# liron88/HM-16.2

Measured on AMD Instinct MI355X. Metric: CTUs/sec (enc) at 4K main10; bit-exact CU partition vs HM, higher is better.
Workload: dtype int32+f64

## Files before the change

### hm-16.2_amd/csrc/hm355_core.h

```cpp
#pragma once
#include <stddef.h>
#include "hm355_types.h"

#ifdef HM355_HOSTSIM
#include <string.h>
#include <math.h>
#include <stdlib.h>
#define HM_DEV static
#define HM_NOINLINE __attribute__((noinline))
#define HM_CONST static const
#define HM_ASSUME_LDS(p) ((void)0)
#define HM_ASSUME_GLB(p) ((void)0)
#define HM_NT 1
static inline int hm_lane() { return 0; }
#define HM_SYNC() ((void)0)
static inline uint32_t hm_wave_sum(uint32_t v) { return v; }
static inline int hm_wave_sum_i(int v) { return v; }
static inline int hm_wave_max_i(int v) { return v; }
#define HM_UNI(x) (x)
#define HM_UCALL(x) (x)
#define hm_uni_ptr(p) (p)
#define hm_uni_struct(v) (v)
#define HM_ENTRY(e) ((void)0)
#define HM_LDS_ADD(p, v) (*(p) += (v))
// ... 206 lines not shown
};
struct CuFrame { int16_t cuZ; int8_t phase, sub, boundary, parentPart, ampSens, pad_; double bestCost, splitCost; uint32_t bestBits, bestDist, splitBits, splitDist; };
struct MvFieldD { MvD mv; int ref; };
struct MergeList { MvFieldD f[5][2]; uint8_t dir[5]; int num; };
struct AmvpInfo { MvD cand[3]; int n; };
struct TZ {
  const Pel *org; int orgStride, w, h;
  const Pel *ref; int refStride;
  uint32_t bestSad; int bestX, bestY, bestDist, bestRound, pointNr;
  int16_t l, r, t, b;
  int16_t subShift, pad_;
  int16_t lx[16], ly[16]; int8_t lp[16], ld[16];
  int16_t wx0, wy0, ww, wh;
};
struct IrqFrame {
  TU t; int8_t phase, child, checkFull, checkSplit, zero; uint8_t bestTS[3];
  uint32_t absSum[3], bestCBF[3], singleBits, singleDist, subBits, subDist; double singleCost, subCost;
};

#define HM_TSTRIDE 33
#define HM_RQ_LDS 256
struct RqLds {
  int32_t lvl[HM_RQ_LDS];
  uint16_t pos[HM_RQ_LDS];
  uint16_t dec[HM_RQ_LDS];
  int16_t cur[HM_RQ_LDS];
  uint8_t ctxSig[HM_RQ_LDS];
  uint8_t code[HM_RQ_LDS];
  uint8_t cgCtxSet[64];
  uint8_t cgFlag[64];
};
struct RefLds {
  Pel refTop[2][132], refLeft[2][132];
  Pel refMain[200], refSide[200];
  Pel line[272];
};
#define HM_SLOT(d, ci) ((d) * CI_NUM + (ci) - ((d) == 4 ? 2 : 0))
#define HM_NUM_SLOTS (4 * CI_NUM + 3)
struct Team;
#define HM_CTU_WAVES 12
struct LdsTables {
  int8_t tmat[32 * HM_TSTRIDE];
  int8_t dst4[16];
  int32_t ebits[128];
};
#if defined(HM355_HOSTSIM)
static LdsTables g_lt;
#else
__shared__ LdsTables g_lt;
#endif
#define HM_LT() (&g_lt)
struct Shared {
  Cabac cur;
  int32_t bufA[32 * HM_TSTRIDE];
  union {
    int32_t bufB[32 * HM_TSTRIDE];
    RqLds rq;
    RefLds ref;
  } u;
  TuWalk walkOuter, walkInner;
  CuFrame cuf[4];
  double outCost; uint32_t outBits, outDist; double outRdCost;
  int32_t mpmZ;
  int32_t s8Winner, s8Reuse;
  InterMeta *im;
  uint32_t mcost; MvD mvPredictor; int32_t costScale;
  union {
    struct {
      uint8_t flags[72];
      RqtFrame rqt[4]; uint32_t rqtRetDist[5], rqtRetBits[5]; double rqtRetCost[5];
      int32_t rdModeList[12];
      uint8_t splitCbf[5][2];
      uint32_t outDistY;
      uint32_t satd[36];
      int32_t mpmNum, mpmPreds[3];
    };
    struct {
      int32_t absCoeff[10];
      TZ tz; MvD outMv; MergeList ml; AmvpInfo amvp; MvFieldD mrgField[2]; int32_t mrgDir, mrgIdx; uint32_t mrgCost, irqZeroDist;
      IrqFrame irq[4];
    };
  };
  int32_t width, height, bitDepth, wCtu, stride[3];
  const Params *P; FrameBuf fb; WorkSpace *ws; const Tables *tab;
  CtuMeta meta;
  TCoeff *cc;
  int32_t ctuX, ctuY, ctuAddr;
// ... 7 lines not shown
static FILE *g_hm_trace;
#define HM_TRACE(e, tag, a, b, c) do { if (g_hm_trace) fprintf(g_hm_trace, "%d %d %u %u %.3f\n", (int)(tag), (e)->ctuAddr, (unsigned)(a), (unsigned)(b), (double)(c)); } while (0)
#elif defined(HM355_TRACE)
#define HM_TRACE_CAP (1u << 21)
__device__ inline void hm_trace(Shared *e, int tag, uint32_t a, uint32_t b, double c)
{
  if (hm_lane() == 0) {
    unsigned long long *t = e->P->prof; const unsigned long long n = atomicAdd(t, 1ull);
    if (n < HM_TRACE_CAP) { t[1 + n * 3] = ((unsigned long long)(uint32_t)tag << 32) | (uint32_t)e->ctuAddr; t[2 + n * 3] = ((unsigned long long)a << 32) | b; t[3 + n * 3] = (unsigned long long)__double_as_longlong(c); }
  }
}
#define HM_TRACE(e, tag, a, b, c) hm_trace((e), (tag), (uint32_t)(a), (uint32_t)(b), (double)(c))
#else
#define HM_TRACE(e, tag, a, b, c) ((void)0)
#endif

#ifndef HM355_HOSTSIM
__shared__ Shared g_sh;
__shared__ Shared g_shs[HM_CTU_WAVES];
#endif
#if !defined(HM355_PROFILE)
static_assert(HM_CTU_WAVES * (sizeof(Shared) + 16) + sizeof(LdsTables) <= 163840 / (12 / HM_CTU_WAVES) && sizeof(Shared) % 8 == 0, "two workgroups of HM_CTU_WAVES searches (+ work items, + the shared tables) per CU: 12 CTU searches in 160 KB of LDS");
#endif
static_assert(offsetof(Shared, bufA) % 8 == 0 && (16 * HM_TSTRIDE * 4) % 8 == 0, "the RDOQ cost array aliases the lower half of bufA as doubles");
static_assert(offsetof(Shared, u) == offsetof(Shared, bufA) + sizeof(((Shared *)0)->bufA), "the motion search stages its reference window across bufA and the union behind it");
#define HM_TZ_WIN_SAMPLES ((int)((sizeof(((Shared *)0)->bufA) + sizeof(((Shared *)0)->u)) / sizeof(Pel)))

HM_DEV inline int hm_clip3(int lo, int hi, int v) { return v < lo ? lo : (v > hi ? hi : v); }
HM_DEV inline int hm_abs(int v) { return v < 0 ? -v : v; }
HM_DEV inline int hm_z2r(int z)
{
  const int x = (z & 1) | ((z >> 1) & 2) | ((z >> 2) & 4) | ((z >> 3) & 8);
  const int y = ((z >> 1) & 1) | ((z >> 2) & 2) | ((z >> 3) & 4) | ((z >> 4) & 8);
  return (y << 4) | x;
}
HM_DEV inline int hm_spread4(int v) { return (v & 1) | ((v & 2) << 1) | ((v & 4) << 2) | ((v & 8) << 3); }
HM_DEV inline int hm_r2z(int r) { return hm_spread4(r & 15) | (hm_spread4(r >> 4) << 1); }
HM_DEV inline int hm_log2(int n) { return n >= 64 ? 6 : (n >= 32 ? 5 : (n >= 16 ? 4 : (n >= 8 ? 3 : 2))); }

HM_DEV inline void par_set8(uint8_t *p, int v, int n) { HM_PAR_FOR(i, n) p[i] = (uint8_t)v; HM_SYNC(); }
HM_DEV inline void par_copy8(uint8_t *d, const uint8_t *s, int n) { HM_PAR_FOR(i, n) d[i] = s[i]; HM_SYNC(); }
HM_DEV inline void par_copy32(TCoeff *d, const TCoeff *s, int n) { HM_PAR_FOR(i, n) d[i] = s[i]; HM_SYNC(); }
HM_DEV inline void par_zero32(TCoeff *d, int n) { HM_PAR_FOR(i, n) d[i] = 0; HM_SYNC(); }
HM_DEV inline void par_copy_blk(Pel *d, int ds, const Pel *s, int ss, int n)
{
  const int l2 = hm_log2(n);
// ... 666 lines not shown
  const uint16_t *scan = e->tab->scan[scanType][log2n - 2], *scanCG = e->tab->scanCG[scanType][log2n - 2];
  const int firstCtx = first_sig_ctx(n, scanType, chroma);
  const int sigOff = C_SIG + (chroma ? 28 : 0);
  const int32_t *src = e->bufA;
  WorkSpace *ws = e->ws;
  const bool big = n == 32;
  double *costCoeff = big ? ws->costCoeff : (double *)(e->bufA + 16 * HM_TSTRIDE);
  int32_t *rqLvl = big ? (int32_t *)e->u.bufB : e->u.rq.lvl;
  uint16_t *rqPos = big ? (uint16_t *)e->bufA : e->u.rq.pos, *rqDec = big ? (uint16_t *)e->bufA + 1024 : e->u.rq.dec;
  int16_t *rqCur = e->u.rq.cur;
  uint8_t *rqCtxSig = e->u.rq.ctxSig, *rqCode = e->u.rq.code;
  uint8_t *cgCtxSet = big ? (uint8_t *)e->u.bufB + 4096 : e->u.rq.cgCtxSet;
  int lastLocal = -1;
  {
    const int64_t cap = 2147483647LL - (1LL << (qBits - 1));
    HM_PAR_FOR(sp, numCoef) {
      const int blkPos = scan[sp];
      const int32_t sc = src[(blkPos >> log2n) * HM_TSTRIDE + (blkPos & (n - 1))];
      const int64_t tmpLevel = (int64_t)hm_abs(sc) * quantCoef;
      const int32_t lvl = (int32_t)(tmpLevel < cap ? tmpLevel : cap);
      rqLvl[sp] = (big && sc < 0) ? ~lvl : lvl;
      if (!big) rqPos[sp] = (uint16_t)(blkPos | (sc < 0 ? 0x8000 : 0));
      if (((lvl + (1 << (qBits - 1))) >> qBits) > 0 && sp > lastLocal) lastLocal = sp;
      dst[sp] = 0;
    }
  }
  const int lastScanPos = hm_wave_max_i(lastLocal);
  HM_SYNC();
  if (big && lastScanPos >= 0) {
    HM_PAR_FOR(sp, numCoef) {
      const int32_t v = rqLvl[sp]; const int neg = v < 0;
      rqLvl[sp] = neg ? ~v : v;
      rqPos[sp] = (uint16_t)(scan[sp] | (neg ? 0x8000 : 0));
      rqDec[sp] = 0;
    }
    HM_SYNC();
  }
  if (lastScanPos < 0) return 0;
  int lastOff, lastShift; last_ctx_params(chroma, n, &lastOff, &lastShift);
  HM_LV(int32_t, tSig); HM_LV(int32_t, tOne); HM_LV(int32_t, tLast); HM_LV(int32_t, tMisc); HM_LV(int32_t, tLastCost);
  HM_LV(double, vCGSig);
  HM_WAVE_FOR(k) {
    const int bin = k & 1, c = k >> 1;
    HM_LVK(tSig, k) = c < (chroma ? 16 : 28) ? HM_LT()->ebits[cb->s[sigOff + c] ^ bin] : 0;
    HM_LVK(tOne, k) = c < 30 ? HM_LT()->ebits[cb->s[C_ONE + c] ^ bin] : 0;
    HM_LVK(tLast, k) = c < 30 ? HM_LT()->ebits[cb->s[(c < 15 ? C_LASTX + c : C_LASTY + c - 15) + (chroma ? 15 : 0)] ^ bin] : 0;
    HM_LVK(tMisc, k) = c < 15 ? HM_LT()->ebits[cb->s[c < 4 ? C_SIG_CG + c : (c < 14 ? C_QT_CBF + c - 4 : C_ROOT_CBF)] ^ bin] : 0;
    HM_LVK(tLastCost, k) = 0;
    HM_LVK(vCGSig, k) = 0;
  }
  {
    const int gmax = HM_GROUP_IDX[n - 1];
    int accX = 0, accY = 0;
    for (int g = 0; g <= gmax; g++) {
      const int cx = (lastOff + (g >> lastShift)) * 2, cy = 30 + cx;
      int bx = accX, by = accY;
      if (g < gmax) { bx += HM_LV_GET(tLast, cx); by += HM_LV_GET(tLast, cy); }
      if (g > 3) { bx += 32768 * ((g - 2) >> 1); by += 32768 * ((g - 2) >> 1); }
      HM_LV_SET(tLastCost, g, bx); HM_LV_SET(tLastCost, 16 + g, by);
      accX += HM_LV_GET(tLast, cx + 1); accY += HM_LV_GET(tLast, cy + 1);
    }
// ... 238 lines not shown
              if (lastCG == 1 && lastNZ == k && hm_abs(dv) == 1) costDown -= (4 << 15);
              if (costUp < costDown) { curCost = costUp; curChange = 1; }
              else { curChange = -1; if (k == firstNZ && hm_abs(dv) == 1) curCost = I64MAX; else curCost = costDown; }
            } else {
              curCost = rdFactor * (-(hm_abs(deltaU))) + (1 << 15) + rateIncUp + sigRateDelta;
              curChange = 1;
              if (k < firstNZ) { const uint32_t thissign = (uint32_t)HM_LV_GET(sNeg, k); if (thissign != signbit) curCost = I64MAX; }
            }
            if (curCost < minCostInc) { minCostInc = curCost; finalChange = curChange; minK = k; }
          }
          if (minK >= 0) {
            const int mv = HM_LV_GET(sCur, minK);
            if (mv == 32767 || mv == -32768) finalChange = -1;
            const int nv = HM_LV_GET(sNeg, minK) ? mv - finalChange : mv + finalChange;
            if (big) HM_LV_SET(sCur, minK, nv); else rqCur[subPos + minK] = (int16_t)nv;
          }
        }
      }
      if (big) { HM_WAVE_FOR(k) { if (k < 16) rqDec[subPos + k] = (uint16_t)(int16_t)HM_LVK(sCur, k); } }
      if (lastCG == 1) lastCG = 0;
    }
  }
  HM_SYNC();
  HM_PAR_FOR(sp, lastScanPos + 1) {
    int v;
    if (!big) v = rqCur[sp];
    else if (absSum >= 2) v = (int16_t)rqDec[sp];
    else { const int lv = (sp < bestLastIdxP1 && ((cgMask >> scanCG[sp >> 4]) & 1)) ? (int)rqDec[sp] : 0; v = (rqPos[sp] & 0x8000) ? -lv : lv; }
    dst[rqPos[sp] & 0x3ff] = v;
  }
  HM_SYNC();
  return absSum;
}

struct CabacR { HM_LV(int32_t, st); HM_LV(int32_t, eb0); HM_LV(int32_t, eb1); HM_LV(int32_t, lps); uint64_t frac; };
HM_DEV inline void cabr_load(const Shared *e, CabacR &r, const Cabac *c)
{
  HM_WAVE_FOR(k) {
    HM_LVK(r.st, k) = k < (int)(sizeof(c->s) / 4) ? ((const int32_t *)c->s)[k] : 0;
    HM_LVK(r.eb0, k) = HM_LT()->ebits[k]; HM_LVK(r.eb1, k) = HM_LT()->ebits[64 + k];
    HM_LVK(r.lps, k) = ((const int32_t *)HM_NEXT_LPS)[k & 31];
  }
  r.frac = c->frac;
}
HM_DEV inline void cabr_store(const CabacR &r, Cabac *c)
{
// ... 1 lines not shown
  c->frac = r.frac;
  HM_SYNC();
}
HM_DEV inline void enc_bin(const Shared *e, CabacR *r, int ctx, int bin)
{
  const int w = HM_LV_GET(r->st, ctx >> 2), sh = (ctx & 3) * 8, s = (w >> sh) & 0xff, i = s ^ bin;
  const int b0 = HM_LV_GET(r->eb0, i & 63), b1 = HM_LV_GET(r->eb1, i & 63);
  r->frac += (uint64_t)(uint32_t)(i < 64 ? b0 : b1);
  const int lw = HM_LV_GET(r->lps, s >> 2);
  const int ns = (bin == (s & 1)) ? (s < 124 ? s + 2 : s) : ((lw >> ((s & 3) * 8)) & 0xff);
  HM_LV_SET(r->st, ctx >> 2, (w & ~(0xff << sh)) | (ns << sh));
}
HM_DEV inline void enc_ep(CabacR *r, int n) { r->frac += (uint64_t)32768 * (uint64_t)n; }
HM_DEV inline void enc_epv(Cabac *c, uint32_t val, int n) { (void)val; enc_ep(c, n); }
HM_DEV inline void enc_epv(CabacR *r, uint32_t val, int n) { (void)val; enc_ep(r, n); }
#include "hm355_bits.h"
HM_DEV inline int hm_min_in_group(int g) { return g < 4 ? g : ((2 + (g & 1)) << ((g >> 1) - 1)); }

#if defined(HM355_PROFILE) && !defined(HM355_HOSTSIM)
#define HM_BPROF(id) do { if (real) { const unsigned long long t_ = __builtin_readcyclecounter(); e->prof[id] += t_ - profT1; e->profCnt[id] += 1; profT1 = t_; } } while (0)
#else
#define HM_BPROF(id) ((void)0)
#endif
template <class C> HM_DEV HM_NOINLINE void code_coeff_nxn(Shared *e, C *c, const TCoeff *coef, int n, int comp, int scanType, int tskipFlag)
{
  HM_ENTRY(e); n = HM_UNI(n); comp = HM_UNI(comp); scanType = HM_UNI(scanType); tskipFlag = HM_UNI(tskipFlag); c = hm_uni_ptr(c); HM_ASSUME_LDS(c); coef = hm_uni_ptr(coef);
  const int chroma = comp != 0, log2n = hm_log2(n), wg = n >> 2;
  const bool real = EngOf<C>::REAL != 0;
#if defined(HM355_PROFILE) && !defined(HM355_HOSTSIM)
  const unsigned long long profT0 = __builtin_readcyclecounter();
#endif
  typename EngOf<C>::R r; cabr_load(e, r, c);
  if (n == 4) enc_bin(e, &r, C_TSKIP + chroma, tskipFlag);
  const uint16_t *scan = e->tab->scan[scanType][log2n - 2], *scanCG = e->tab->scanCG[scanType][log2n - 2];
  int16_t *lv = (n == 32) ? (int16_t *)e->bufA : e->u.rq.cur; uint8_t *cgFlag = e->u.rq.cgFlag;
  uint16_t *sposArr = (n == 32) ? (uint16_t *)e->bufA + 1024 : e->u.rq.pos;
  HM_PAR_FOR(i, 64) cgFlag[i] = 0;
  HM_SYNC();
  int lastLocal = -1;
  HM_PAR_FOR(sp, n * n) {
    const int blkPos = scan[sp]; const TCoeff v = coef[blkPos];
    lv[sp] = (int16_t)v; sposArr[sp] = (uint16_t)blkPos;
    if (v != 0) { if (sp > lastLocal) lastLocal = sp; const int py = blkPos >> log2n, px = blkPos - (py << log2n); cgFlag[wg * (py >> 2) + (px >> 2)] = 1; }
  }
  const int scanPosLast = hm_wave_max_i(lastLocal);
  HM_SYNC();
#if defined(HM355_PROFILE) && !defined(HM355_HOSTSIM)
  if (real) { e->prof[PR_ADI] += __builtin_readcyclecounter() - profT0; e->profCnt[PR_ADI] += 1; }
  unsigned long long profT1 = __builtin_readcyclecounter();
#endif
  uint64_t cgMask = 0;
  HM_LV(int32_t, vScanCG);
  HM_WAVE_FOR(k) { HM_BALLOT(cgMask, k, cgFlag[k] != 0); HM_LVK(vScanCG, k) = k < wg * wg ? scanCG[k] : 0; }
  const int posLast = sposArr[scanPosLast];
  {
    int py = posLast >> log2n, px = posLast - (py << log2n);
    if (scanType == SCAN_VER) { const int t = px; px = py; py = t; }
    const int gx = hm_group_idx(px), gy = hm_group_idx(py), gmax = hm_group_idx(n - 1);
    int off, shift; last_ctx_params(chroma, n, &off, &shift);
    const int bxc = C_LASTX + (chroma ? 15 : 0) + off, byc = C_LASTY + (chroma ? 15 : 0) + off;
    int k;
    for (k = 0; k < gx; k++) enc_bin(e, &r, bxc + (k >> shift), 1);
    if (gx < gmax) enc_bin(e, &r, bxc + (k >> shift), 0);
    for (k = 0; k < gy; k++) enc_bin(e, &r, byc + (k >> shift), 1);
    if (gy < gmax) enc_bin(e, &r, byc + (k >> shift), 0);
    if (gx > 3) enc_epv(&r, (uint32_t)(px - hm_min_in_group(gx)), (gx - 2) >> 1);
    if (gy > 3) enc_epv(&r, (uint32_t)(py - hm_min_in_group(gy)), (gy - 2) >> 1);
  }
  HM_BPROF(PR_INV);
  const int firstCtx = first_sig_ctx(n, scanType, chroma), sigOff = C_SIG + (chroma ? 28 : 0);
  const int lastScanSet = scanPosLast >> 4;
  int c1 = 1;
  for (int subSet = lastScanSet; subSet >= 0; subSet--) {
    const int subPos = subSet << 4, isLastSet = subSet == lastScanSet;
    const int cgBlkPos = HM_LV_GET(vScanCG, subSet), cgy = cgBlkPos >> (log2n - 2), cgx = cgBlkPos & (wg - 1);
    const int sigRight = (cgx < wg - 1) ? (int)((cgMask >> (cgBlkPos + 1)) & 1) : 0;
    const int sigLower = (cgy < wg - 1) ? (int)((cgMask >> (cgBlkPos + wg)) & 1) : 0;
    if (isLastSet || subSet == 0) cgMask |= 1ull << cgBlkPos;
    else enc_bin(e, &r, C_SIG_CG + (chroma ? 2 : 0) + ((sigRight + sigLower) != 0), (int)((cgMask >> cgBlkPos) & 1));
    if (!((cgMask >> cgBlkPos) & 1)) continue;
    const int pattern = wg <= 1 ? 0 : sigRight + (sigLower << 1);
    const int top = isLastSet ? (scanPosLast & 15) : 15;
    HM_LV(int32_t, vCtx); HM_LV(int32_t, vAbs);
    uint64_t nz = 0, g1 = 0, g2 = 0, ng = 0;
    HM_WAVE_FOR(k) {
      const int kk = k & 15, sp = subPos + kk;
      const int a = (kk <= top) ? hm_abs((int)lv[sp]) : 0;
      if (real) HM_BALLOT(ng, k, kk <= top && lv[sp] < 0 && k < 16);
      HM_LVK(vAbs, k) = a;
      HM_LVK(vCtx, k) = sig_ctx_inc(pattern, firstCtx, sposArr[sp], log2n, chroma);
      HM_BALLOT(nz, k, a != 0 && k < 16); HM_BALLOT(g1, k, a > 1 && k < 16); HM_BALLOT(g2, k, a > 2 && k < 16);
    }
    HM_BPROF(PR_SATD35);
    {
      int seen = isLastSet ? 1 : 0;
      for (int p = isLastSet ? top - 1 : 15; p >= 0; p--) {
        const int sig = (int)((nz >> p) & 1);
        if (p > 0 || subSet == 0 || seen) enc_bin(e, &r, sigOff + HM_LV_GET(vCtx, p), sig);
        seen += sig;
      }
    }
    HM_BPROF(PR_TUBLK);
    const int numNonZero = __builtin_popcountll(nz);
    if (numNonZero > 0) {
      const int lastNZ = 63 - __builtin_clzll(nz), firstNZ = __builtin_ctzll(nz);
      const int signHidden = (lastNZ - firstNZ >= 4);
      const int ctxSet = ctx_set_index(chroma, subSet, c1 == 0);
      c1 = 1;
      int firstC2 = -1, escape = 0, idx = 0;
      for (uint64_t m = nz; m && idx < 8; idx++) {
        const int p = 63 - __builtin_clzll(m); m &= ~(1ull << p);
        const int sym = (int)((g1 >> p) & 1);
        enc_bin(e, &r, C_ONE + 4 * ctxSet + c1, sym);
// ... 170 lines not shown
    enc_subdiv_cbf_qt(e, &r, t, bLuma, bChroma);
    cabr_store(r, &e->cur);
  }
  if (bLuma) enc_coeff_qt(e, t, 0);
  if (bChroma) { enc_coeff_qt(e, t, 1); enc_coeff_qt(e, t, 2); }
  HM_PROF_END(e, PR_BITS);
  return num_bits(&e->cur);
}

HM_DEV HM_NOINLINE uint32_t intra_coding_tu_block(Shared *e, TU tv, int comp, int save1load2)
{
  HM_ENTRY(e); comp = HM_UNI(comp); save1load2 = HM_UNI(save1load2); tv = hm_uni_struct(tv);
  const TU *t = &tv;
  CtuMeta *m = (&e->meta); WorkSpace *ws = e->ws;
  if (comp && !t->cW) return 0;
  const int n = comp ? t->cW : (1 << t->log2), l2 = hm_log2(n);
  const int relZ = comp ? t->cRelZ : t->relZ, z = t->cuZ + relZ;
  const int bx = comp ? t->cx : t->x, by = comp ? t->cy : t->y;
  const int st = HM_PLANE_STRIDE(comp), po = HM_PLANE_OFF(comp);
  const int layer = 5 - t->log2, parts = comp ? t->cParts : t->parts;
  const int ps = e->stride[comp], bitDepth = e->bitDepth;
  const Pel *org = e->fb.org[comp] + (e->ctuY * st + by) * ps + e->ctuX * st + bx;
  Pel *recPic = e->fb.rec[comp] + (e->ctuY * st + by) * ps + e->ctuX * st + bx;
  Pel *pred = ws->pred + po + by * st + bx, *resi = ws->resi + po + by * st + bx;
  Pel *recQt = ws->qtRec[layer] + po + by * st + bx;
  TCoeff *coef = ws->qtCoef[layer] + po + (comp ? t->cOff : z * 16);
  const int tskip = m->ts[comp][z];
  int mode = comp ? m->dirC[z] : m->dirL[z];
  if (comp && mode == DM_CHROMA_IDX) mode = m->dirL[z & ~3];
  if (save1load2 != 2) {
    const int filt = use_filtered_refs(comp, mode, n);
    const int r = hm_z2r(z);
    { HM_PROF_BEGIN(e, PR_ADI); init_adi_pattern(e, comp, e->ctuX * st + bx, e->ctuY * st + by, n, e->ctuX * 16 + (r & 15), e->ctuY * 16 + (r >> 4), comp ? n / 2 : n / 4, filt); HM_PROF_END(e, PR_ADI); }
    { HM_PROF_BEGIN(e, PR_PRED); pred_intra(e, comp, mode, n, filt, pred, st); HM_PROF_END(e, PR_PRED); }
    if (save1load2 == 1) { HM_PAR_FOR(i, 16) e->ws->tsPred[comp][i] = pred[(i >> 2) * st + (i & 3)]; HM_SYNC(); }
  } else { HM_PAR_FOR(i, 16) pred[(i >> 2) * st + (i & 3)] = e->ws->tsPred[comp][i]; HM_SYNC(); }
  if (comp == 0) par_set8(m->tr + z, t->trDepth, parts);
  const int tshift = 15 - bitDepth - l2;
  HM_PAR_FOR(i, n * n) {
    const int y = i >> l2, x = i & (n - 1);
    const int r = org[y * ps + x] - pred[y * st + x];
    resi[y * st + x] = (Pel)r;
    e->bufA[y * HM_TSTRIDE + x] = tskip ? (r << tshift) : r;
  }
  HM_SYNC();
  { HM_PROF_BEGIN(e, PR_FWD); if (!tskip) fwd_transform(e, n, comp == 0 && n == 4, bitDepth); HM_PROF_END(e, PR_FWD); }
  const int cbfCtx = comp ? 5 + t->trDepth : (t->trDepth == 0 ? 1 : 0);
  HM_PROF_BEGIN(e, PR_RDOQ);
  const int absSum = rdoq_is_empty(e, n, comp) ? 0 : (int)HM_UCALL(rdoq(e, coef, n, comp, coef_scan_idx(m, z, n, comp), cbfCtx));
  HM_PROF_END(e, PR_RDOQ);
#if defined(HM355_PROFILE) && !defined(HM355_HOSTSIM)
  { const int pid = l2 == 2 ? (absSum ? 13 : 7) : (l2 == 3 ? 14 : (l2 == 4 ? 15 : 43)); e->prof[pid] += __builtin_readcyclecounter() - prof_t0_PR_RDOQ; e->profCnt[pid] += 1; }
#endif
  par_set8(m->cbf[comp] + z, (absSum > 0 ? 1 : 0) << t->trDepth, parts);
  HM_PROF_BEGIN(e, PR_INV);
  if (absSum > 0) {
    const int rightShift = 6 - (tshift + e->fb.qpPer[comp != 0]);
    const int scale = HM_INV_QUANT_SCALES[e->fb.qpRem[comp != 0]];
    int tgt = 25 + rightShift; if (tgt > 16) tgt = 16;
    const int imin = -(1 << (tgt - 1)), imax = (1 << (tgt - 1)) - 1;
    HM_PAR_FOR(i, n * n) {
      const int y = i >> l2, x = i & (n - 1);
      const int c = hm_clip3(imin, imax, coef[i]);
      int v;
      if (rightShift > 0) v = (c * scale + (1 << (rightShift - 1))) >> rightShift;
      else v = (int)((unsigned)(c * scale) << (-rightShift));
      e->bufA[y * HM_TSTRIDE + x] = hm_clip3(-32768, 32767, v);
    }
    HM_SYNC();
    if (!tskip) inv_transform(e, n, comp == 0 && n == 4, bitDepth);
    const int off = tshift == 0 ? 0 : (1 << (tshift - 1));
    HM_PAR_FOR(i, n * n) {
      const int y = i >> l2, x = i & (n - 1);
      const int v = e->bufA[y * HM_TSTRIDE + x];
      resi[y * st + x] = (Pel)(tskip ? ((v + off) >> tshift) : v);
    }
  } else {
    HM_PAR_FOR(i, n * n) { const int y = i >> l2, x = i & (n - 1); coef[i] = 0; resi[y * st + x] = 0; }
  }
  HM_SYNC();
  HM_PROF_END(e, PR_INV);
  const int maxv = (1 << bitDepth) - 1, shiftSse = (bitDepth - 8) << 1;
  uint32_t sse = 0;
  HM_PAR_FOR(i, n * n) {
    const int y = i >> l2, x = i & (n - 1);
    const int r = hm_clip3(0, maxv, pred[y * st + x] + resi[y * st + x]);
    pred[y * st + x] = (Pel)r; recQt[y * st + x] = (Pel)r; recPic[y * ps + x] = (Pel)r;
    const int d = org[y * ps + x] - r; sse += (uint32_t)((d * d) >> shiftSse);
  }
  uint32_t d = hm_wave_sum(sse);
  HM_SYNC();
  if (comp) d = (uint32_t)(e->fb.chromaWeight * (double)d);
  return d;
}

HM_DEV inline void store_intra_result_qt(Shared *e, const TU *t, int comp)
{
  const int st = HM_PLANE_STRIDE(comp), po = HM_PLANE_OFF(comp), layer = 5 - t->log2;
  const int bx = comp ? t->cx : t->x, by = comp ? t->cy : t->y;
  const TCoeff *coef = e->ws->qtCoef[layer] + po + (comp ? t->cOff : (t->cuZ + t->relZ) * 16);
  const Pel *rq = e->ws->qtRec[layer] + po + by * st + bx;
  HM_PAR_FOR(i, 16) { e->ws->tsCoef[comp][i] = coef[i]; e->ws->tsRec[comp][i] = rq[(i >> 2) * st + (i & 3)]; }
  HM_SYNC();
}
HM_DEV inline void load_intra_result_qt(Shared *e, const TU *t, int comp)
{
  const int st = HM_PLANE_STRIDE(comp), po = HM_PLANE_OFF(comp), layer = 5 - t->log2, ps = e->stride[comp];
  const int bx = comp ? t->cx : t->x, by = comp ? t->cy : t->y;
  TCoeff *coef = e->ws->qtCoef[layer] + po + (comp ? t->cOff : (t->cuZ + t->relZ) * 16);
  Pel *rq = e->ws->qtRec[layer] + po + by * st + bx;
  Pel *recPic = e->fb.rec[comp] + (e->ctuY * st + by) * ps + e->ctuX * st + bx;
  HM_PAR_FOR(i, 16) { coef[i] = e->ws->tsCoef[comp][i]; const Pel v = e->ws->tsRec[comp][i]; rq[(i >> 2) * st + (i & 3)] = v; recPic[(i >> 2) * ps + (i & 3)] = v; }
  HM_SYNC();
}

HM_DEV HM_NOINLINE void simt4_luma_leaf(Shared *e, TU tv);
// ... 4 lines not shown
  CtuMeta *m = (&e->meta);
  RqtFrame *fr = e->rqt; int sp = 0;
  uint32_t *retDist = e->rqtRetDist, *retBits = e->rqtRetBits; double *retCost = e->rqtRetCost;
  fr[0].t = rootv; fr[0].phase = 0; retDist[0] = 0; retBits[0] = 0; retCost[0] = 0.0;
  while (sp >= 0) {
    RqtFrame *f = &fr[sp]; const TU *t = &f->t;
    const int z = t->cuZ + t->relZ, fullDepth = t->cuDepth + t->trDepth, log2 = t->log2;
    if (f->phase == 0) {
      const int nxn = m->part[t->cuZ] == SIZE_NxN;
      f->checkFull = log2 <= 5;
      f->checkSplit = log2 > tr_min_size_in_cu(6 - t->cuDepth, nxn);
      if (checkFirst && f->checkFull) f->checkSplit = 0;
      f->singleCost = HM_MAX_DOUBLE; f->singleDist = 0; f->singleCbf = 0; f->bestModeId = 0; f->singleBits = 0;
      const int checkTS = (log2 == 2) && (m->part[z] == SIZE_NxN);
      if (f->checkFull) {
        if (checkTS) {
          cabac_copy(&e->ws->slot[HM_SLOT(fullDepth, CI_QT_TRAFO_ROOT)], &e->cur);
          for (int modeId = 0; modeId < 2; modeId++) {
            double costTmp;
            par_set8(m->ts[0] + z, modeId, t->parts);
            const uint32_t distTmp = HM_UCALL(intra_coding_tu_block(e, *t, 0, modeId == 0 ? 1 : 2));
            const uint32_t cbfTmp = (m->cbf[0][z] >> t->trDepth) & 1;
            if (modeId == 1 && cbfTmp == 0) costTmp = HM_MAX_DOUBLE;
            else { const uint32_t bits = HM_UCALL(intra_bits_qt(e, *t, 1, 0)); costTmp = calc_rd_cost(e, bits, distTmp); }
            if (costTmp < f->singleCost) {
              f->singleCost = costTmp; f->singleDist = distTmp; f->singleCbf = cbfTmp; f->bestModeId = (int8_t)modeId;
              if (modeId == 0) { store_intra_result_qt(e, t, 0); cabac_copy(&e->ws->slot[HM_SLOT(fullDepth, CI_TEMP_BEST)], &e->cur); }
            }
            if (modeId == 0) cabac_copy(&e->cur, &e->ws->slot[HM_SLOT(fullDepth, CI_QT_TRAFO_ROOT)]);
          }
          par_set8(m->ts[0] + z, f->bestModeId, t->parts);
          if (f->bestModeId == 0) {
            load_intra_result_qt(e, t, 0);
            par_set8(m->cbf[0] + z, (int)(f->singleCbf << t->trDepth), t->parts);
            cabac_copy(&e->cur, &e->ws->slot[HM_SLOT(fullDepth, CI_TEMP_BEST)]);
          }
        } else if (log2 == 2 && e->P->fewWaves) {
          par_set8(m->ts[0] + z, 0, t->parts);
          HM_PROF_BEGIN(e, PR_S4LEAF);
          simt4_luma_leaf(e, *t);
          HM_PROF_END(e, PR_S4LEAF);
          f->singleDist = e->outDistY; f->singleBits = e->outBits;
          f->singleCost = calc_rd_cost(e, e->outBits, f->singleDist);
        } else if (sp == 0 && e->s8Reuse == 1) {
          e->s8Reuse = 0;
          cabac_copy(&e->ws->slot[HM_SLOT(fullDepth, CI_QT_TRAFO_ROOT)], &e->cur);
          par_set8(m->ts[0] + z, 0, t->parts);
// ... 1 lines not shown
          simt8_luma_winner_as_single_tu(e, *t);
          f->singleDist = e->outDistY; f->singleCbf = e->outDist;
          par_set8(m->cbf[0] + z, (int)(f->singleCbf << t->trDepth), t->parts);
          f->singleCost = calc_rd_cost(e, e->outBits, f->singleDist);
        } else if (sp == 0 && e->s8Reuse == 2) {
          e->s8Reuse = 0;
          cabac_copy(&e->ws->slot[HM_SLOT(fullDepth, CI_QT_TRAFO_ROOT)], &e->cur);
          par_set8(m->ts[0] + z, 0, t->parts);
          par_set8(m->tr + z, t->trDepth, t->parts);
          {
            const int n = 1 << log2, layer = 5 - log2;
            par_copy32(e->ws->qtCoef[layer] + z * 16, e->cc + z * 16, n * n);
            par_copy_blk(e->ws->qtRec[layer] + t->y * 64 + t->x, 64, e->ws->reco + t->y * 64 + t->x, 64, n);
          }
          f->singleCbf = e->ws->tmpCbf[0][0] & 1;
          par_set8(m->cbf[0] + z, (int)(f->singleCbf << t->trDepth), t->parts);
          f->singleDist = e->outDistY; f->singleCost = e->outRdCost;
          cabac_copy(&e->cur, &e->ws->slot[HM_SLOT(fullDepth, CI_QT_TRAFO_TEST)]);
        } else {
          if (f->checkSplit) cabac_copy(&e->ws->slot[HM_SLOT(fullDepth, CI_QT_TRAFO_ROOT)], &e->cur);
          par_set8(m->ts[0] + z, 0, t->parts);
          f->singleDist = HM_UCALL(intra_coding_tu_block(e, *t, 0, 0));
          if (f->checkSplit) f->singleCbf = (m->cbf[0][z] >> t->trDepth) & 1;
          const uint32_t bits = HM_UCALL(intra_bits_qt(e, *t, 1, 0));
          f->singleCost = calc_rd_cost(e, bits, f->singleDist); f->singleBits = bits;
        }
      }
      if (!f->checkSplit) { retDist[sp] += f->singleDist; retBits[sp] += f->singleBits; retCost[sp] += f->singleCost; sp--; continue; }
      if (f->checkFull) { cabac_copy(&e->ws->slot[HM_SLOT(fullDepth, CI_QT_TRAFO_TEST)], &e->cur); cabac_copy(&e->cur, &e->ws->slot[HM_SLOT(fullDepth, CI_QT_TRAFO_ROOT)]); }
      else cabac_copy(&e->ws->slot[HM_SLOT(fullDepth, CI_QT_TRAFO_ROOT)], &e->cur);
      f->splitCost = 0.0; f->splitDist = 0; f->splitCbf = 0; f->child = 0; f->phase = 1;
      retDist[sp + 1] = 0; retBits[sp + 1] = 0; retCost[sp + 1] = 0.0;
    }
    if (f->phase == 1) {
      int splitLost = 0;
      if (f->child > 0) {
        const TU ch = tu_child(t, f->child - 1, 0);
        f->splitCbf |= (m->cbf[0][ch.cuZ + ch.relZ] >> ch.trDepth) & 1;
        const uint32_t lbBits = retBits[sp + 1] > (uint32_t)f->child ? retBits[sp + 1] - (uint32_t)f->child : 0;
        if (f->checkFull) splitLost = !(calc_rd_cost(e, lbBits, retDist[sp + 1]) < f->singleCost);
        else if (sp == 0 && !(calc_rd_cost(e, lbBits, retDist[1]) < e->outCost)) {
          e->outDistY = 0; e->outRdCost = HM_MAX_DOUBLE; return;
        }
      }
      if (!splitLost) {
        if (f->child < 4) {
// ... 161 lines not shown
  const int fullDepth = t->cuDepth + t->trDepth;
  int checkTS = (t->cW == 4) && (t->log2 == 2);
  if (checkTS) { int nb = 0; for (int s = 0; s < 4; s++) nb += m->ts[0][z + s]; checkTS = nb > 0; }
  const int zc = t->cuZ + t->cRelZ;
  if (t->cW == 4 && !checkTS) {
    cabac_copy(&e->ws->slot[HM_SLOT(fullDepth, CI_QT_TRAFO_ROOT)], &e->cur);
    HM_PROF_BEGIN(e, PR_S4CLEAF);
    const uint32_t d2 = HM_UCALL(simt4_chroma_leaf(e, *t));
    HM_PROF_END(e, PR_S4CLEAF);
    return d2;
  }
  uint32_t dist = 0;
  for (int comp = 1; comp < 3; comp++) {
    cabac_copy(&e->ws->slot[HM_SLOT(fullDepth, CI_QT_TRAFO_ROOT)], &e->cur);
    double singleCost = HM_MAX_DOUBLE, costTmp = 0; uint32_t singleDistC = 0, singleCbfC = 0; int bestTS = 0, bestModeId = 0, currModeId = 0;
    const int total = checkTS ? 2 : 1;
    for (int tsMode = 0; tsMode < total; tsMode++) {
      par_set8(m->ts[comp] + zc, tsMode, t->cParts);
      currModeId++;
      const int isOne = (total == 1), isLast = (currModeId == total);
      const uint32_t distTmp = HM_UCALL(intra_coding_tu_block(e, *t, comp, isOne ? 0 : (tsMode == 0 ? 1 : 2)));
      const uint32_t cbfTmp = (m->cbf[comp][zc] >> t->trDepth) & 1;
      if (tsMode == 1 && cbfTmp == 0) costTmp = HM_MAX_DOUBLE;
      else if (!isOne) { reset_bits(&e->cur); enc_coeff_qt(e, t, comp); costTmp = calc_rd_cost(e, num_bits(&e->cur), distTmp); }
      if (costTmp < singleCost) {
        singleCost = costTmp; singleDistC = distTmp; bestTS = tsMode; bestModeId = currModeId; singleCbfC = cbfTmp;
        if (!isOne && !isLast) { store_intra_result_qt(e, t, comp); cabac_copy(&e->ws->slot[HM_SLOT(fullDepth, CI_TEMP_BEST)], &e->cur); }
      }
      if (!isOne && !isLast) cabac_copy(&e->cur, &e->ws->slot[HM_SLOT(fullDepth, CI_QT_TRAFO_ROOT)]);
    }
    if (bestModeId < total) {
      load_intra_result_qt(e, t, comp);
      par_set8(m->cbf[comp] + zc, (int)(singleCbfC << t->trDepth), t->cParts);
      cabac_copy(&e->cur, &e->ws->slot[HM_SLOT(fullDepth, CI_TEMP_BEST)]);
    }
    par_set8(m->ts[comp] + zc, bestTS, t->cParts);
    dist += singleDistC;
  }
  return dist;
}
HM_DEV HM_NOINLINE uint32_t recur_intra_chroma_coding_qt(Shared *e, TU rootv)
{
  HM_ENTRY(e); rootv = hm_uni_struct(rootv);
  const TU *root = &rootv;
  CtuMeta *m = (&e->meta);
  uint32_t dist = 0;
  TuWalk &w = e->walkOuter; walk_begin(&w, root);
// ... 387 lines not shown
      if (inside && depth != 3) enc_bin(e, c, C_SPLIT + ctx_split_flag(e, z, depth), m->depth[z] > depth);
      if (!((depth < m->depth[z] && depth < 3) || !inside)) {
        if (m->pred[z] == MODE_INTER) encode_cu_syntax_inter(e, c, z, depth, 1); else encode_cu_syntax(e, c, z, depth);
        const int lastX = ((lx + size) % 64 == 0) || (lx + size == e->width), lastY = ((ty + size) % 64 == 0) || (ty + size == e->height);
        if (lastX && lastY && !lastCtuOfSlice) enc_trm(e, c, 0);
        sp--; continue;
      }
      stackNext[sp] = 0;
    }
    if (stackNext[sp] == 4) { sp--; continue; }
    const int s = stackNext[sp]++;
    const int q = (256 >> (2 * depth)) >> 2, sz = z + s * q, rr = hm_z2r(sz);
    const int sx = e->ctuX * 64 + (rr & 15) * 4, sy = e->ctuY * 64 + (rr >> 4) * 4;
    if (sx < e->width && sy < e->height) { stackZ[sp + 1] = (int16_t)sz; stackNext[sp + 1] = -1; sp++; }
  }
}

#if !defined(HM355_HOSTSIM)
#include "hm355_team.h"
#endif
HM_DEV inline void process_ctu(Shared *e, const Params *P, const WorkItem *it, int wsIndex, Team *team = 0)
{
  e->P = P; e->fb = P->frames[it->frame]; e->ws = P->ws + wsIndex; e->tab = P->tab;
  e->width = P->width; e->height = P->height; e->bitDepth = P->bitDepth; e->wCtu = P->wCtu; e->mpmZ = -1; e->s8Reuse = 0;
  for (int c = 0; c < 3; c++) e->stride[c] = P->stride[c];
  e->ctuX = it->ctuX; e->ctuY = it->ctuY; e->ctuAddr = it->ctuY * P->wCtu + it->ctuX;
  e->cc = e->fb.coef + (size_t)e->ctuAddr * HM_COEF_CTU;
  e->im = e->fb.imeta ? e->fb.imeta + e->ctuAddr : (InterMeta *)0;
  HM_SYNC();
  if (e->im) {
    const int bnd = it->ctuX * 64 + 63 >= P->width || it->ctuY * 64 + 63 >= P->height;
    const MvD *src = e->ctuAddr == 0 ? e->fb.ip->integerMv2Nx2N[0] : e->fb.intMv + (size_t)(e->ctuAddr - 1) * 32;
    HM_PAR_FOR(i, 32) { MvD v; v.x = v.y = 0; if (bnd) v = src[i]; e->ws->intMv[i >> 4][i & 15] = v; }
    HM_SYNC();
  }
#if defined(HM355_PROFILE) && !defined(HM355_HOSTSIM)
  for (int i = 0; i < HM_PROF_N; i++) { e->prof[i] = 0; e->profCnt[i] = 0; }
#endif
  HM_PROF_BEGIN(e, PR_TOTAL);
#if defined(HM355_HOSTSIM)
  load_tables();
#endif
  const int a = e->ctuAddr, numCtus = P->wCtu * P->hCtu;
  {
    CtuMeta *m = (&e->meta);
    HM_PAR_FOR(z, 256) {
      m->depth[z] = 0; m->part[z] = SIZE_NONE; m->pred[z] = MODE_NONE; m->dirL[z] = DC_IDX; m->dirC[z] = 0; m->tr[z] = 0;
// ... 70 lines not shown
```

### hm-16.2_amd/csrc/hm355_team.h

```cpp
#pragma once

#define HM_TEAM 9
#define HM_TEAM_I 5
#define HM_TEAM_HELPERS 4
#define HM_TEAM_TIMEOUT_TICKS (20ull * 100000000ull)
enum { TK_INTRA = 0, TK_CHAIN = 1, TK_PAIR1 = 2, TK_PAIR2 = 3 };

struct TeamBox {
  uint32_t reqSeq, doneSeq;
  int32_t cuZ, depth, part, kind;
  int32_t src, sens, owner, improved;
  uint32_t bits, dist; double cost;
  double threshold;
};
struct Team {
  TeamBox box[HM_TEAM - 1];
  uint32_t quit, dead;
  unsigned int *abortWord;
  WorkItem item;
  int32_t waves, pad_[3];
  Shared sh[1];
};
static_assert(offsetof(Team, sh) % 16 == 0, "Shared holds doubles and 16-byte rows");
#define HM_TEAM_LDS_BYTES(waves) (offsetof(Team, sh) + (size_t)(waves) * sizeof(Shared))
// ... 336 lines not shown
        f->splitBits += num_bits(&e->cur);
      }
      f->splitCost = calc_rd_cost(e, f->splitBits, f->splitDist);
      cabac_copy(&e->ws->slot[HM_SLOT(cuDepth, CI_TEMP_BEST)], &e->ws->slot[HM_SLOT(cuDepth + 1, CI_NEXT_BEST)]);
      if (f->splitCost < f->bestCost) {
        f->bestCost = f->splitCost; f->bestBits = f->splitBits; f->bestDist = f->splitDist;
        cabac_copy(&e->ws->slot[HM_SLOT(cuDepth, CI_NEXT_BEST)], &e->ws->slot[HM_SLOT(cuDepth, CI_TEMP_BEST)]);
      } else team_take_unsplit(e, cuDepth, cuZ, cuDepth);
      if (sp > 0 && !f->boundary) sensitive[sp - 1] |= HM_UNI(HM_TEAM_PTR()->box[cuDepth].sens);
      retCost = f->bestCost; retBits = f->bestBits; retDist = f->bestDist; sp--; continue;
    }
    if (f->phase == 2) { f->splitBits += retBits; f->splitDist += retDist; f->phase = 1; continue; }
  }
  HM_TSTAT_T1(1, tAll); HM_TSTAT_ADD(0, 1);
  e->outCost = retCost; e->outBits = retBits; e->outDist = retDist;
}

HM_DEV inline void team_adopt(Shared *e, const Shared *src, int wave, Pel *win)
{
  e->P = src->P; e->fb = src->fb; e->tab = src->tab;
  e->width = src->width; e->height = src->height; e->bitDepth = src->bitDepth; e->wCtu = src->wCtu;
  for (int c = 0; c < 3; c++) e->stride[c] = src->stride[c];
  e->ctuX = src->ctuX; e->ctuY = src->ctuY; e->ctuAddr = src->ctuAddr;
  e->ws = team_wave_ws(wave); e->cc = e->ws->teamCoef; e->im = (InterMeta *)0; e->mpmZ = -1; e->s8Reuse = 0;
  if (e->fb.dqp && hm_lane() == 0) e->ws->dq = src->ws->dq;
  if (win) {
    Pel *w = win;
    for (int c = 0; c < 3; c++) {
      const int S = c ? 32 : 64;
      e->fb.rec[c] = w - ((long long)e->ctuY * S - 1) * e->stride[c];
      w += (size_t)(S + 1) * e->stride[c];
    }
  }
  HM_SYNC();
}
HM_DEV inline void team_fill_window(Shared *e, const Shared *mainSh)
{
  for (int c = 0; c < 3; c++) {
    const int S = c ? 32 : 64, ps = e->stride[c];
    const int x0 = e->ctuX * S > 0 ? e->ctuX * S - 1 : 0, x1 = (e->ctuX + 2) * S < ps ? (e->ctuX + 2) * S : ps;
    const int y0 = e->ctuY > 0 ? e->ctuY * S - 1 : 0, y1 = (e->ctuY + 1) * S, w = x1 - x0;
    const Pel *src = mainSh->fb.rec[c]; Pel *dst = e->fb.rec[c];
    HM_PAR_FOR_XY(x, y, w, w * (y1 - y0)) dst[(size_t)(y0 + y) * ps + x0 + x] = src[(size_t)(y0 + y) * ps + x0 + x];
  }
  HM_SYNC();
}
HM_DEV inline void team_copy_arrays(Shared *e, const Shared *src)
// ... 77 lines not shown
```

Measured before the change: 25200.

## Keep small-TU prediction and RDOQ scan-order levels in LDS for coefficient coding

```diff
diff --git a/hm-16.2_amd/csrc/hm355_core.h b/hm-16.2_amd/csrc/hm355_core.h
--- a/hm-16.2_amd/csrc/hm355_core.h
+++ b/hm-16.2_amd/csrc/hm355_core.h
@@ -252,14 +252,15 @@
 #define HM_RQ_LDS 256
 struct RqLds {
   int32_t lvl[HM_RQ_LDS];
-  uint16_t pos[HM_RQ_LDS];
   uint16_t dec[HM_RQ_LDS];
-  int16_t cur[HM_RQ_LDS];
   uint8_t ctxSig[HM_RQ_LDS];
   uint8_t code[HM_RQ_LDS];
   uint8_t cgCtxSet[64];
   uint8_t cgFlag[64];
+  int16_t cur[HM_RQ_LDS];
+  uint16_t pos[HM_RQ_LDS];
 };
+struct TuLds { uint8_t rq_[sizeof(RqLds)]; Pel pred[HM_RQ_LDS]; };
 struct RefLds {
   Pel refTop[2][132], refLeft[2][132];
   Pel refMain[200], refSide[200];
@@ -287,12 +288,14 @@
     int32_t bufB[32 * HM_TSTRIDE];
     RqLds rq;
     RefLds ref;
+    TuLds tu;
   } u;
   TuWalk walkOuter, walkInner;
   CuFrame cuf[4];
   double outCost; uint32_t outBits, outDist; double outRdCost;
   int32_t mpmZ;
   int32_t s8Winner, s8Reuse;
+  uint32_t rqTag;
   InterMeta *im;
   uint32_t mcost; MvD mvPredictor; int32_t costScale;
   union {
@@ -346,6 +349,8 @@
 #if !defined(HM355_PROFILE)
 static_assert(HM_CTU_WAVES * (sizeof(Shared) + 16) + sizeof(LdsTables) <= 163840 / (12 / HM_CTU_WAVES) && sizeof(Shared) % 8 == 0, "two workgroups of HM_CTU_WAVES searches (+ work items, + the shared tables) per CU: 12 CTU searches in 160 KB of LDS");
 #endif
+static_assert(offsetof(Shared, im) == offsetof(Shared, rqTag) + 4, "rqTag takes padding, not room");
+static_assert(offsetof(RqLds, cur) >= 16 * HM_TSTRIDE * 4 && sizeof(TuLds) <= sizeof(((Shared *)0)->u), "the scan-order levels and the prediction of a block up to 16x16 lie behind its transform temp, inside the union");
 static_assert(offsetof(Shared, bufA) % 8 == 0 && (16 * HM_TSTRIDE * 4) % 8 == 0, "the RDOQ cost array aliases the lower half of bufA as doubles");
 static_assert(offsetof(Shared, u) == offsetof(Shared, bufA) + sizeof(((Shared *)0)->bufA), "the motion search stages its reference window across bufA and the union behind it");
 #define HM_TZ_WIN_SAMPLES ((int)((sizeof(((Shared *)0)->bufA) + sizeof(((Shared *)0)->u)) / sizeof(Pel)))
@@ -1058,7 +1063,7 @@
       rqLvl[sp] = (big && sc < 0) ? ~lvl : lvl;
       if (!big) rqPos[sp] = (uint16_t)(blkPos | (sc < 0 ? 0x8000 : 0));
       if (((lvl + (1 << (qBits - 1))) >> qBits) > 0 && sp > lastLocal) lastLocal = sp;
-      dst[sp] = 0;
+      if (dst) dst[sp] = 0;
     }
   }
   const int lastScanPos = hm_wave_max_i(lastLocal);
@@ -1073,6 +1078,7 @@
     HM_SYNC();
   }
   if (lastScanPos < 0) return 0;
+  if (!dst) { HM_PAR_FOR(i, numCoef) e->bufA[(i >> log2n) * HM_TSTRIDE + (i & (n - 1))] = 0; }
   int lastOff, lastShift; last_ctx_params(chroma, n, &lastOff, &lastShift);
   HM_LV(int32_t, tSig); HM_LV(int32_t, tOne); HM_LV(int32_t, tLast); HM_LV(int32_t, tMisc); HM_LV(int32_t, tLastCost);
   HM_LV(double, vCGSig);
@@ -1357,6 +1363,14 @@
     }
   }
   HM_SYNC();
+  if (!dst) {
+    HM_PAR_FOR(sp, numCoef) {
+      if (sp <= lastScanPos) { const int blkPos = rqPos[sp] & 0x3ff; e->bufA[(blkPos >> log2n) * HM_TSTRIDE + (blkPos & (n - 1))] = rqCur[sp]; }
+      else rqCur[sp] = 0;
+    }
+    HM_SYNC();
+    return absSum;
+  }
   HM_PAR_FOR(sp, lastScanPos + 1) {
     int v;
     if (!big) v = rqCur[sp];
@@ -1404,6 +1418,7 @@
 #else
 #define HM_BPROF(id) ((void)0)
 #endif
+HM_DEV inline uint32_t rq_tag(const TCoeff *coef, int tskip) { return (uint32_t)(size_t)coef | (tskip ? 2u : 0u) | 1u; }
 template <class C> HM_DEV HM_NOINLINE void code_coeff_nxn(Shared *e, C *c, const TCoeff *coef, int n, int comp, int scanType, int tskipFlag)
 {
   HM_ENTRY(e); n = HM_UNI(n); comp = HM_UNI(comp); scanType = HM_UNI(scanType); tskipFlag = HM_UNI(tskipFlag); c = hm_uni_ptr(c); HM_ASSUME_LDS(c); coef = hm_uni_ptr(coef);
@@ -1417,13 +1432,21 @@
   const uint16_t *scan = e->tab->scan[scanType][log2n - 2], *scanCG = e->tab->scanCG[scanType][log2n - 2];
   int16_t *lv = (n == 32) ? (int16_t *)e->bufA : e->u.rq.cur; uint8_t *cgFlag = e->u.rq.cgFlag;
   uint16_t *sposArr = (n == 32) ? (uint16_t *)e->bufA + 1024 : e->u.rq.pos;
+  bool onChip = false;
+  if (!real) { onChip = n <= 16 && (uint32_t)HM_UNI(e->rqTag) == rq_tag(coef, tskipFlag); e->rqTag = 0; }
   HM_PAR_FOR(i, 64) cgFlag[i] = 0;
   HM_SYNC();
   int lastLocal = -1;
-  HM_PAR_FOR(sp, n * n) {
-    const int blkPos = scan[sp]; const TCoeff v = coef[blkPos];
-    lv[sp] = (int16_t)v; sposArr[sp] = (uint16_t)blkPos;
-    if (v != 0) { if (sp > lastLocal) lastLocal = sp; const int py = blkPos >> log2n, px = blkPos - (py << log2n); cgFlag[wg * (py >> 2) + (px >> 2)] = 1; }
+  if (onChip) {
+    HM_PAR_FOR(sp, n * n) {
+      if (lv[sp] != 0) { if (sp > lastLocal) lastLocal = sp; const int blkPos = sposArr[sp] & 0x3ff, py = blkPos >> log2n, px = blkPos - (py << log2n); cgFlag[wg * (py >> 2) + (px >> 2)] = 1; }
+    }
+  } else {
+    HM_PAR_FOR(sp, n * n) {
+      const int blkPos = scan[sp]; const TCoeff v = coef[blkPos];
+      lv[sp] = (int16_t)v; sposArr[sp] = (uint16_t)blkPos;
+      if (v != 0) { if (sp > lastLocal) lastLocal = sp; const int py = blkPos >> log2n, px = blkPos - (py << log2n); cgFlag[wg * (py >> 2) + (px >> 2)] = 1; }
+    }
   }
   const int scanPosLast = hm_wave_max_i(lastLocal);
   HM_SYNC();
@@ -1434,7 +1457,7 @@
   uint64_t cgMask = 0;
   HM_LV(int32_t, vScanCG);
   HM_WAVE_FOR(k) { HM_BALLOT(cgMask, k, cgFlag[k] != 0); HM_LVK(vScanCG, k) = k < wg * wg ? scanCG[k] : 0; }
-  const int posLast = sposArr[scanPosLast];
+  const int posLast = sposArr[scanPosLast] & 0x3ff;
   {
     int py = posLast >> log2n, px = posLast - (py << log2n);
     if (scanType == SCAN_VER) { const int t = px; px = py; py = t; }
@@ -1470,7 +1493,7 @@
       const int a = (kk <= top) ? hm_abs((int)lv[sp]) : 0;
       if (real) HM_BALLOT(ng, k, kk <= top && lv[sp] < 0 && k < 16);
       HM_LVK(vAbs, k) = a;
-      HM_LVK(vCtx, k) = sig_ctx_inc(pattern, firstCtx, sposArr[sp], log2n, chroma);
+      HM_LVK(vCtx, k) = sig_ctx_inc(pattern, firstCtx, sposArr[sp] & 0x3ff, log2n, chroma);
       HM_BALLOT(nz, k, a != 0 && k < 16); HM_BALLOT(g1, k, a > 1 && k < 16); HM_BALLOT(g2, k, a > 2 && k < 16);
     }
     HM_BPROF(PR_SATD35);
@@ -1687,32 +1710,35 @@
   const int ps = e->stride[comp], bitDepth = e->bitDepth;
   const Pel *org = e->fb.org[comp] + (e->ctuY * st + by) * ps + e->ctuX * st + bx;
   Pel *recPic = e->fb.rec[comp] + (e->ctuY * st + by) * ps + e->ctuX * st + bx;
-  Pel *pred = ws->pred + po + by * st + bx, *resi = ws->resi + po + by * st + bx;
+  const bool small = n <= 16;
+  Pel *pred = small ? e->u.tu.pred : ws->pred + po + by * st + bx;
+  const int pst = small ? n : st;
   Pel *recQt = ws->qtRec[layer] + po + by * st + bx;
   TCoeff *coef = ws->qtCoef[layer] + po + (comp ? t->cOff : z * 16);
   const int tskip = m->ts[comp][z];
   int mode = comp ? m->dirC[z] : m->dirL[z];
   if (comp && mode == DM_CHROMA_IDX) mode = m->dirL[z & ~3];
+  e->rqTag = 0;
   if (save1load2 != 2) {
     const int filt = use_filtered_refs(comp, mode, n);
     const int r = hm_z2r(z);
     { HM_PROF_BEGIN(e, PR_ADI); init_adi_pattern(e, comp, e->ctuX * st + bx, e->ctuY * st + by, n, e->ctuX * 16 + (r & 15), e->ctuY * 16 + (r >> 4), comp ? n / 2 : n / 4, filt); HM_PROF_END(e, PR_ADI); }
-    { HM_PROF_BEGIN(e, PR_PRED); pred_intra(e, comp, mode, n, filt, pred, st); HM_PROF_END(e, PR_PRED); }
-    if (save1load2 == 1) { HM_PAR_FOR(i, 16) e->ws->tsPred[comp][i] = pred[(i >> 2) * st + (i & 3)]; HM_SYNC(); }
-  } else { HM_PAR_FOR(i, 16) pred[(i >> 2) * st + (i & 3)] = e->ws->tsPred[comp][i]; HM_SYNC(); }
+    { HM_PROF_BEGIN(e, PR_PRED); pred_intra(e, comp, mode, n, filt, pred, pst); HM_PROF_END(e, PR_PRED); }
+    if (save1load2 == 1) { HM_PAR_FOR(i, 16) e->ws->tsPred[comp][i] = pred[i]; HM_SYNC(); }
+  } else { HM_PAR_FOR(i, 16) pred[i] = e->ws->tsPred[comp][i]; HM_SYNC(); }
   if (comp == 0) par_set8(m->tr + z, t->trDepth, parts);
   const int tshift = 15 - bitDepth - l2;
   HM_PAR_FOR(i, n * n) {
     const int y = i >> l2, x = i & (n - 1);
-    const int r = org[y * ps + x] - pred[y * st + x];
-    resi[y * st + x] = (Pel)r;
+    const int r = org[y * ps + x] - pred[y * pst + x];
     e->bufA[y * HM_TSTRIDE + x] = tskip ? (r << tshift) : r;
   }
   HM_SYNC();
   { HM_PROF_BEGIN(e, PR_FWD); if (!tskip) fwd_transform(e, n, comp == 0 && n == 4, bitDepth); HM_PROF_END(e, PR_FWD); }
   const int cbfCtx = comp ? 5 + t->trDepth : (t->trDepth == 0 ? 1 : 0);
   HM_PROF_BEGIN(e, PR_RDOQ);
-  const int absSum = rdoq_is_empty(e, n, comp) ? 0 : (int)HM_UCALL(rdoq(e, coef, n, comp, coef_scan_idx(m, z, n, comp), cbfCtx));
+  const int searched = !rdoq_is_empty(e, n, comp);
+  const int absSum = searched ? (int)HM_UCALL(rdoq(e, small ? (TCoeff *)0 : coef, n, comp, coef_scan_idx(m, z, n, comp), cbfCtx)) : 0;
   HM_PROF_END(e, PR_RDOQ);
 #if defined(HM355_PROFILE) && !defined(HM355_HOSTSIM)
   { const int pid = l2 == 2 ? (absSum ? 13 : 7) : (l2 == 3 ? 14 : (l2 == 4 ? 15 : 43)); e->prof[pid] += __builtin_readcyclecounter() - prof_t0_PR_RDOQ; e->profCnt[pid] += 1; }
@@ -1726,7 +1752,9 @@
     const int imin = -(1 << (tgt - 1)), imax = (1 << (tgt - 1)) - 1;
     HM_PAR_FOR(i, n * n) {
       const int y = i >> l2, x = i & (n - 1);
-      const int c = hm_clip3(imin, imax, coef[i]);
+      int lv;
+      if (small) { lv = e->bufA[y * HM_TSTRIDE + x]; coef[i] = lv; } else lv = coef[i];
+      const int c = hm_clip3(imin, imax, lv);
       int v;
       if (rightShift > 0) v = (c * scale + (1 << (rightShift - 1))) >> rightShift;
       else v = (int)((unsigned)(c * scale) << (-rightShift));
@@ -1734,29 +1762,31 @@
     }
     HM_SYNC();
     if (!tskip) inv_transform(e, n, comp == 0 && n == 4, bitDepth);
-    const int off = tshift == 0 ? 0 : (1 << (tshift - 1));
-    HM_PAR_FOR(i, n * n) {
-      const int y = i >> l2, x = i & (n - 1);
-      const int v = e->bufA[y * HM_TSTRIDE + x];
-      resi[y * st + x] = (Pel)(tskip ? ((v + off) >> tshift) : v);
-    }
-  } else {
-    HM_PAR_FOR(i, n * n) { const int y = i >> l2, x = i & (n - 1); coef[i] = 0; resi[y * st + x] = 0; }
-  }
-  HM_SYNC();
+  } else if (small || !searched) {
+    HM_PAR_FOR(i, n * n) coef[i] = 0;
+  }
   HM_PROF_END(e, PR_INV);
   const int maxv = (1 << bitDepth) - 1, shiftSse = (bitDepth - 8) << 1;
+  const int off = tshift == 0 ? 0 : (1 << (tshift - 1));
   uint32_t sse = 0;
   HM_PAR_FOR(i, n * n) {
     const int y = i >> l2, x = i & (n - 1);
-    const int r = hm_clip3(0, maxv, pred[y * st + x] + resi[y * st + x]);
-    pred[y * st + x] = (Pel)r; recQt[y * st + x] = (Pel)r; recPic[y * ps + x] = (Pel)r;
+    int rs = 0;
+    if (absSum > 0) { const int v = e->bufA[y * HM_TSTRIDE + x]; rs = (Pel)(tskip ? ((v + off) >> tshift) : v); }
+    const int r = hm_clip3(0, maxv, pred[y * pst + x] + rs);
+    recQt[y * st + x] = (Pel)r; recPic[y * ps + x] = (Pel)r;
     const int d = org[y * ps + x] - r; sse += (uint32_t)((d * d) >> shiftSse);
   }
   uint32_t d = hm_wave_sum(sse);
   HM_SYNC();
   if (comp) d = (uint32_t)(e->fb.chromaWeight * (double)d);
   return d;
+}
+HM_DEV inline void rq_tag_set(Shared *e, const TU *t, int comp)
+{
+  const int z = t->cuZ + (comp ? t->cRelZ : t->relZ), n = comp ? t->cW : (1 << t->log2);
+  if (n <= 16 && (((&e->meta)->cbf[comp][z] >> t->trDepth) & 1))
+    e->rqTag = rq_tag(e->ws->qtCoef[5 - t->log2] + HM_PLANE_OFF(comp) + (comp ? t->cOff : z * 16), (&e->meta)->ts[comp][z]);
 }
 
 HM_DEV inline void store_intra_result_qt(Shared *e, const TU *t, int comp)
@@ -1807,7 +1837,7 @@
             const uint32_t distTmp = HM_UCALL(intra_coding_tu_block(e, *t, 0, modeId == 0 ? 1 : 2));
             const uint32_t cbfTmp = (m->cbf[0][z] >> t->trDepth) & 1;
             if (modeId == 1 && cbfTmp == 0) costTmp = HM_MAX_DOUBLE;
-            else { const uint32_t bits = HM_UCALL(intra_bits_qt(e, *t, 1, 0)); costTmp = calc_rd_cost(e, bits, distTmp); }
+            else { rq_tag_set(e, t, 0); const uint32_t bits = HM_UCALL(intra_bits_qt(e, *t, 1, 0)); costTmp = calc_rd_cost(e, bits, distTmp); }
             if (costTmp < f->singleCost) {
               f->singleCost = costTmp; f->singleDist = distTmp; f->singleCbf = cbfTmp; f->bestModeId = (int8_t)modeId;
               if (modeId == 0) { store_intra_result_qt(e, t, 0); cabac_copy(&e->ws->slot[HM_SLOT(fullDepth, CI_TEMP_BEST)], &e->cur); }
@@ -1855,6 +1885,7 @@
           par_set8(m->ts[0] + z, 0, t->parts);
           f->singleDist = HM_UCALL(intra_coding_tu_block(e, *t, 0, 0));
           if (f->checkSplit) f->singleCbf = (m->cbf[0][z] >> t->trDepth) & 1;
+          rq_tag_set(e, t, 0);
           const uint32_t bits = HM_UCALL(intra_bits_qt(e, *t, 1, 0));
           f->singleCost = calc_rd_cost(e, bits, f->singleDist); f->singleBits = bits;
         }
@@ -2062,7 +2093,7 @@
       const uint32_t distTmp = HM_UCALL(intra_coding_tu_block(e, *t, comp, isOne ? 0 : (tsMode == 0 ? 1 : 2)));
       const uint32_t cbfTmp = (m->cbf[comp][zc] >> t->trDepth) & 1;
       if (tsMode == 1 && cbfTmp == 0) costTmp = HM_MAX_DOUBLE;
-      else if (!isOne) { reset_bits(&e->cur); enc_coeff_qt(e, t, comp); costTmp = calc_rd_cost(e, num_bits(&e->cur), distTmp); }
+      else if (!isOne) { rq_tag_set(e, t, comp); reset_bits(&e->cur); enc_coeff_qt(e, t, comp); costTmp = calc_rd_cost(e, num_bits(&e->cur), distTmp); }
       if (costTmp < singleCost) {
         singleCost = costTmp; singleDistC = distTmp; bestTS = tsMode; bestModeId = currModeId; singleCbfC = cbfTmp;
         if (!isOne && !isLast) { store_intra_result_qt(e, t, comp); cabac_copy(&e->ws->slot[HM_SLOT(fullDepth, CI_TEMP_BEST)], &e->cur); }
@@ -2496,7 +2527,7 @@
 HM_DEV inline void process_ctu(Shared *e, const Params *P, const WorkItem *it, int wsIndex, Team *team = 0)
 {
   e->P = P; e->fb = P->frames[it->frame]; e->ws = P->ws + wsIndex; e->tab = P->tab;
-  e->width = P->width; e->height = P->height; e->bitDepth = P->bitDepth; e->wCtu = P->wCtu; e->mpmZ = -1; e->s8Reuse = 0;
+  e->width = P->width; e->height = P->height; e->bitDepth = P->bitDepth; e->wCtu = P->wCtu; e->mpmZ = -1; e->s8Reuse = 0; e->rqTag = 0;
   for (int c = 0; c < 3; c++) e->stride[c] = P->stride[c];
   e->ctuX = it->ctuX; e->ctuY = it->ctuY; e->ctuAddr = it->ctuY * P->wCtu + it->ctuX;
   e->cc = e->fb.coef + (size_t)e->ctuAddr * HM_COEF_CTU;
diff --git a/hm-16.2_amd/csrc/hm355_team.h b/hm-16.2_amd/csrc/hm355_team.h
--- a/hm-16.2_amd/csrc/hm355_team.h
+++ b/hm-16.2_amd/csrc/hm355_team.h
@@ -382,7 +382,7 @@
   e->width = src->width; e->height = src->height; e->bitDepth = src->bitDepth; e->wCtu = src->wCtu;
   for (int c = 0; c < 3; c++) e->stride[c] = src->stride[c];
   e->ctuX = src->ctuX; e->ctuY = src->ctuY; e->ctuAddr = src->ctuAddr;
-  e->ws = team_wave_ws(wave); e->cc = e->ws->teamCoef; e->im = (InterMeta *)0; e->mpmZ = -1; e->s8Reuse = 0;
+  e->ws = team_wave_ws(wave); e->cc = e->ws->teamCoef; e->im = (InterMeta *)0; e->mpmZ = -1; e->s8Reuse = 0; e->rqTag = 0;
   if (e->fb.dqp && hm_lane() == 0) e->ws->dq = src->ws->dq;
   if (win) {
     Pel *w = win;
```

Measured after the change: 25230, median of 6. No clear change (+0.1%).
